# ZackAttack614/BlackBird

Measured on AMD Instinct MI355X. Metric: selfplay_games_per_sec, higher is better.
Workload: dtype f32 (float32 operands split exactly into 3 bf16 values, 6 bf16 MFMA products each, f32 accumulate)

## Files before the change

blackbird_amd/csrc/mega2.hip.h:

```cpp
#pragma once
#include "net.hip.h"
#include "net_x3.hip.h"
#include "tree.hip.h"

#define MEGA_RMAX 4
#define MEGA_HEAD_FLOATS 192

#define MEGA2_QCAP 32
#ifndef BB_TREE_IDLE_SLEEP
#define BB_TREE_IDLE_SLEEP 4
#endif
#ifndef BB_NET_IDLE_SLEEP
#define BB_NET_IDLE_SLEEP 4
#endif

__device__ __forceinline__ int lds_load(volatile int *p) { return *p; }
__device__ __forceinline__ void release_global_then_lds() {
    __threadfence_block();
    asm volatile("s_waitcnt vmcnt(0)" ::: "memory");
}


#define BB_QUEUE_SHADOWED(B, R) BB_SLOTS_TREE(B, B, R) BB_SLOTS_MAILBOX(B, B) BB_SLOTS_RESUME(B)
#define BB_QUEUE_COPY_ORDER(X)                                                                                           \
    X(root) X(root_N) X(n_nodes) X(ply) X(sims_left) X(pend_leaf) X(pend_expand) X(path_len) X(game_lid) X(sim_serial)   \
    X(leaf_serial) X(resume_cur) X(resume_depth) X(leaf_game_id) X(root_W) X(eval_value) X(eval_policy) X(evals) X(ctr)  \
    X(path) X(root_pp) X(leaf_flags)
#define BB_QUEUE_COPY_ORDER_REC(X) X(path_N) X(path_all) X(path_W)
#define BB_COUNT(...) +1
#define BB_SHADOW_PER(f) ((int)(sizeof(f) / sizeof(f[0])) / GW)
template <class G, int GW, bool REC>
struct GameShadow {
    static constexpr int S = G::S, MP = G::MAXPATH, PS = S;
#define X(T, f, per) T f[REC ? GW * (per) : 1];
    BB_QUEUE_SHADOWED(BB_SHADOW_MEMBER, X)
#undef X
    typename G::State leaf_state[GW];
    static_assert(0 BB_QUEUE_COPY_ORDER(BB_COUNT) BB_QUEUE_COPY_ORDER_REC(BB_COUNT) == 0 BB_QUEUE_SHADOWED(BB_COUNT, BB_COUNT), "a row is not copied");
    __device__ __forceinline__ void load(const TreeDev &d, int g0, int n, int nthreads) {
#define X(f) BB_SHADOW_LOAD(d, f, BB_SHADOW_PER(f))
        BB_QUEUE_COPY_ORDER(X)
        if constexpr (REC) { BB_QUEUE_COPY_ORDER_REC(X) }
#undef X
        for (int i = threadIdx.x; i < n; i += nthreads) leaf_state[i] = ((const typename G::State *)d.leaf_state)[g0 + i];
    }
    __device__ __forceinline__ void store(const TreeDev &d, int g0, int n, int nthreads) {
#define X(f) BB_SHADOW_STORE(d, f, BB_SHADOW_PER(f))
        BB_QUEUE_COPY_ORDER(X)
        if constexpr (REC) { BB_QUEUE_COPY_ORDER_REC(X) }
#undef X
        for (int i = threadIdx.x; i < n; i += nthreads) ((typename G::State *)d.leaf_state)[g0 + i] = leaf_state[i];
    }
    __device__ __forceinline__ TreeDev local(const TreeDev &d, int g0) {
        TreeDev r = d;
#define X(f) r.f = f;
        BB_QUEUE_COPY_ORDER(X)
        if constexpr (REC) { BB_QUEUE_COPY_ORDER_REC(X) }
#undef X
        r.leaf_state = leaf_state;
        r.pool_g0 = g0;
        return r;
    }
};

struct QueueCtl {
    int q[MEGA2_QCAP];
    int head, tail, tree_done, abort_flag;
};

__device__ __attribute__((noinline)) int queue_pop(QueueCtl *c, long long t_start, long long t_limit, int n_tree) {
    int li = -1;
    if ((threadIdx.x & 63) == 0) {
        int h = lds_load(&c->head), t = lds_load(&c->tail);
        if (h < t) {
            if (atomicCAS(&c->head, h, h + 1) == h) {
                volatile int *slot = &c->q[h & (MEGA2_QCAP - 1)];
                for (int spin = 0; spin < (1 << 20) && (li = *slot) < 0; spin++) __builtin_amdgcn_s_sleep(1);
                *slot = -1;
                if (li < 0) {
                    c->abort_flag = 1;
                    li = -2;
// ... 296 lines not shown
```

blackbird_amd/csrc/tree.hip.h:

```cpp
#pragma once
#include "games.hip.h"
#include "rng.hip.h"

#define NODE_EXPANDED 1
#define NODE_TERMINAL 2
#define NODE_CACHED 4
#define LEAF_RECORDED 0x40000000
#define CHILD_NONE (-1)
#define CHILD_TERM_BIT 0x40000000

template <class G>
struct alignas(128) DenseNode {
    int32_t flags;
    uint32_t legal_mask;
    int32_t all;
    int32_t serial;
    double sq;
    double pad0;
    int32_t N[G::S];
    float Q[G::S];
    int32_t child[G::S];
    alignas(128) double cP[G::S];
    float W[G::S];
    typename G::State st;
};

struct ExampleHdr {
    uint32_t game_id;
    uint16_t ply;
    uint8_t player;
    int8_t z;
    uint32_t total;
    uint32_t n_children;
};

#define BB_SLOTS_TREE(B, Q, R)                                                                     \
    B(int32_t, root, 1) B(int32_t, root_N, 1) B(int32_t, n_nodes, 1) B(int32_t, ply, 1) B(int32_t, sims_left, 1)           \
    B(int32_t, pend_leaf, 1) B(int32_t, pend_expand, 1) B(int32_t, path_len, 1)                                            \
    B(int32_t, game_lid, 1)                                             \
    B(int32_t, sim_serial, 1) B(float, root_W, 1)                                                                          \
    B(int8_t, root_pp, 1)                                   \
    B(uint32_t, path, MP)                                                                \
        \
    R(int32_t, path_N, MP) R(int32_t, path_all, MP)       \
    R(float, path_W, MP)                                                               \
    Q(int32_t, leaf_flags, 1)
#define BB_SLOTS_ANC(X)                                                                                 \
       \
    X(uint32_t, anc, ANC)                                                                                                   \
    X(int32_t, anc_len, 1) X(int32_t, top_N, 1)
#define BB_SLOTS_MAILBOX(B, Q)                                                 \
    B(uint32_t, leaf_game_id, 1) B(int32_t, leaf_serial, 1) B(float, eval_value, 1) Q(float, eval_policy, PS)              \
    B(uint64_t, evals, 1)                                                              \
    B(uint64_t, ctr, 8)
#define BB_SLOTS_OUT(X)                                                       \
    X(int32_t, out_action, 1) X(int32_t, out_root_plays, 1) X(int32_t, out_child_plays, S)                                 \
    X(float, out_root_winrate, 1) X(float, out_child_value, S)
#define BB_SLOTS_RESUME(X) X(int32_t, resume_cur, 1) X(int32_t, resume_depth, 1)
#define BB_SLOTS_POST(X) X(int, post_slot, 1)
#define BB_ROW_NONE(...)
#define BB_SLOT_ARRAYS(X) BB_SLOTS_TREE(X, X, X) BB_SLOTS_ANC(X) BB_SLOTS_MAILBOX(X, X) BB_SLOTS_OUT(X) BB_SLOTS_RESUME(X) BB_SLOTS_POST(X)
#define BB_SLOT_SHADOWED(X) BB_SLOTS_TREE(X, BB_ROW_NONE, BB_ROW_NONE) BB_SLOTS_MAILBOX(X, BB_ROW_NONE)
#define BB_SLOT_POINTER(T, f, per) T *f;
#define BB_SHADOW_MEMBER(T, f, per) T f[GW * (per)];
#define BB_SHADOW_LOAD(o, f, per) for (int i = threadIdx.x; i < n * (per); i += nthreads) f[i] = o.f[(size_t)g0 * (per) + i];
#define BB_SHADOW_STORE(o, f, per) for (int i = threadIdx.x; i < n * (per); i += nthreads) o.f[(size_t)g0 * (per) + i] = f[i];

struct TreeDev {
    int n_slots, node_cap, sims_per_move, max_plies, kind, max_depth, evaluator, priors_ones;
    int salt_per_game, max_games;
    int gpw;
    double c_puct;
    uint64_t seed, salt;
    uint32_t first_game_id;
    BB_SLOTS_TREE(BB_SLOT_POINTER, BB_SLOT_POINTER, BB_SLOT_POINTER)
    int track_anc;
    BB_SLOTS_ANC(BB_SLOT_POINTER)
    void *leaf_state;
    BB_SLOTS_MAILBOX(BB_SLOT_POINTER, BB_SLOT_POINTER)
    void *nodes;
    int n_games_target;
    double temp;
    uint8_t *examples;
    int32_t *game_hdr;
    int example_bytes;
    BB_SLOTS_OUT(BB_SLOT_POINTER)
    const double *in_u;
    BB_SLOTS_RESUME(BB_SLOT_POINTER)
    int *post_count;
    BB_SLOTS_POST(BB_SLOT_POINTER)
    int level_budget;
    int slot_offset;
    int lid_stride;
    int pool_g0;
    int *visit_pool;
    float noise_alpha;
    void *eval_cache;
    int eval_cache_log2;
// ... 30 lines not shown
#pragma unroll
    for (int k = 0; k < A; k++) a[k] = __shfl(x, k, S);
    if (A < 8) {
        double res = 0.;
#pragma unroll
        for (int k = 0; k < A; k++) res += a[k];
        return res;
    } else {
        double r[8];
#pragma unroll
        for (int j = 0; j < 8; j++) r[j] = a[j];
        int i = 8;
        for (; i < A - (A % 8); i += 8)
            for (int j = 0; j < 8; j++) r[j] += a[i + j];
        double res = ((r[0] + r[1]) + (r[2] + r[3])) + ((r[4] + r[5]) + (r[6] + r[7]));
        for (; i < A; i++) res += a[i];
        return res;
    }
}

template <int S, int STEP>
__device__ __forceinline__ void argmax_step(double &u, int &idx, int &payload) {
    double ou = dpp_step_d<STEP>(u);
    int oi = dpp_step_i<STEP>(idx), op = dpp_step_i<STEP>(payload);
    if (ou > u || (ou == u && oi < idx)) {
        u = ou;
        idx = oi;
        payload = op;
    }
}
template <int S>
__device__ __forceinline__ int grp_argmax(double u, int idx, int &payload) {
    (void)idx;
    double m = u;
    m = __builtin_fmax(m, dpp_step_d<0>(m));
    m = __builtin_fmax(m, dpp_step_d<1>(m));
    m = __builtin_fmax(m, dpp_step_d<2>(m));
    if (S == 16) m = __builtin_fmax(m, dpp_step_d<3>(m));
    const unsigned long long eq = __ballot(u == m);
    const int l64 = (int)__lane_id();
    const unsigned grp = (unsigned)(eq >> (l64 & ~(S - 1))) & ((1u << S) - 1u);
    const int win = __ffs(grp) - 1;
    payload = __shfl(payload, win, S);
    return win;
}

__device__ __forceinline__ double puct_score(double q, double cPi, double sq, int Ni, bool legal) {
    double u = q + __ddiv_rn(cPi * sq, 1.0 + (double)Ni);
    return legal ? u : -1.0;
}
#ifndef BB_PUCT_FILTER
#define BB_PUCT_FILTER 1
#endif
template <int S>
__device__ __forceinline__ int grp_argmax_puct(float qf, double cPi, double sq, int Ni, bool legal, int &payload) {
#if BB_PUCT_FILTER
    const float num = (float)(cPi * sq);
    const float uf = legal ? __builtin_fmaf(num, __builtin_amdgcn_rcpf((float)(Ni + 1)), qf) : -1.0f;
    float mf = uf;
    mf = __builtin_fmaxf(mf, __int_as_float(dpp_step_i<0>(__float_as_int(mf))));
    mf = __builtin_fmaxf(mf, __int_as_float(dpp_step_i<1>(__float_as_int(mf))));
    mf = __builtin_fmaxf(mf, __int_as_float(dpp_step_i<2>(__float_as_int(mf))));
    if (S == 16) mf = __builtin_fmaxf(mf, __int_as_float(dpp_step_i<3>(__float_as_int(mf))));
    const bool mine = uf >= mf - mf * 0x1p-18f && uf >= 0.0f;
    const unsigned long long cand = __ballot(mine);
    const int l64 = (int)__lane_id();
    const unsigned grp = (unsigned)(cand >> (l64 & ~(S - 1))) & ((1u << S) - 1u);
    if (__ballot((grp & (grp - 1u)) != 0u || grp == 0u) == 0ull) {
        const int win = __ffs(grp) - 1;
        int p = mine ? payload : 0;
        p |= dpp_step_i<0>(p);
        p |= dpp_step_i<1>(p);
        p |= dpp_step_i<2>(p);
        if (S == 16) p |= dpp_step_i<3>(p);
        payload = p;
        return win;
    }
#endif
    return grp_argmax<S>(puct_score((double)qf, cPi, sq, Ni, legal), 0, payload);
}
__device__ __forceinline__ double child_q(const TreeDev &d, float Qi, float Wi, int Ni) {
    if (d.evaluator != 2) return (double)Qi;
    return Ni > 0 ? (double)Wi / (double)Ni : 0.0;
}

template <class G>
__device__ __forceinline__ void backup_path(const TreeDev &d, int g, int lane, DenseNode<G> *pool, int plen, float v01,
                                            int prev) {
    constexpr int S = G::S;
    float vflip = 1.0f - v01;
    const uint32_t *path = d.path + (size_t)g * G::MAXPATH;
    auto edge = [&](uint32_t e) __attribute__((always_inline)) {
        int a = e & 15, pl = (e >> 4) & 3;
        DenseNode<G> *pn = pool + (e >> 6);
        int n = pn->N[a] + 1, all = pn->all + 1;
        float w = pn->W[a] + ((pl == prev) ? v01 : vflip);
        pn->N[a] = n;
        pn->W[a] = w;
        pn->Q[a] = __fdiv_rn(w, (float)n);
        pn->all = all;
        pn->sq = __dsqrt_rn(1.0 + (double)all);
    };
    for (int k = lane; k < plen; k += S) edge(path[k]);
    if (d.track_anc) {
        const uint32_t *anc = d.anc + (size_t)g * (d.max_plies + 2);
        const int na = d.anc_len[g];
        for (int k = lane; k < na; k += S) edge(anc[k]);
        if (lane == 0) d.top_N[g] += 1;
    }
    if (lane == 0) {
        d.root_N[g] += 1;
        int pp = d.root_pp[g];
        if (pp) d.root_W[g] += (pp == prev) ? v01 : vflip;
    }
}

template <class G>
__device__ __forceinline__ void phase_apply(const TreeDev &d, int g, int lane) {
    using Node = DenseNode<G>;
    constexpr int S = G::S, A = G::A;
    int leaf = d.pend_leaf[g];
    if (leaf < 0) return;
    Node *pool = (Node *)d.nodes + (size_t)(g + d.pool_g0) * d.node_cap;
    Node *node = pool + leaf;
    typename G::State st = ((const typename G::State *)d.leaf_state)[g];
    float v = d.eval_value[g];
    if (d.pend_expand[g]) {
        uint32_t mask = G::legal_mask(st);
        double x = 0.0;
        if (lane < A) x = (double)d.eval_policy[(size_t)g * S + lane] * (double)((mask >> lane) & 1u);
        double tot = grp_np_sum<A, S>(x);
        node->N[lane] = 0;
        node->Q[lane] = 0.f;
        node->W[lane] = 0.f;
        node->child[lane] = CHILD_NONE;
        node->cP[lane] = (lane < A) ? d.c_puct * __ddiv_rn(x, tot) : 0.0;
        if (lane == 0) {
            node->flags |= NODE_EXPANDED;
            node->legal_mask = mask;
            node->all = 0;
            node->sq = 1.0;
        }
    }
    int player = gs_player(st), prev = gs_prev(st);
    float v01;
    if (d.evaluator == 2) {
        v01 = v;
    } else {
        v01 = (v + 1.0f) * 0.5f;
        if (player != prev) v01 = 1.0f - v01;
    }
    if (d.evaluator != 2 && !d.pend_expand[g] && (node->flags & NODE_TERMINAL) && lane == 0) {
        node->pad0 = (double)v01;
        node->flags |= NODE_CACHED;
    }
    backup_path<G>(d, g, lane, pool, d.path_len[g], v01, prev);
    if (lane == 0) d.pend_leaf[g] = -1;
}

template <class G>
__device__ __forceinline__ void backup_path_rec(const TreeDev &d, int g, int lane, DenseNode<G> *pool, int plen, float v01, int prev) {
    constexpr int S = G::S;
    const float vflip = 1.0f - v01;
    const uint32_t *path = d.path + (size_t)g * G::MAXPATH;
    const int32_t *pN = d.path_N + (size_t)g * G::MAXPATH, *pA = d.path_all + (size_t)g * G::MAXPATH;
    const float *pW = d.path_W + (size_t)g * G::MAXPATH;
    for (int k = lane; k < plen; k += S) {
        const uint32_t e = path[k];
        const int a = e & 15, pl = (e >> 4) & 3;
        DenseNode<G> *pn = pool + (e >> 6);
        const int n = pN[k] + 1, all = pA[k] + 1;
        const float w = pW[k] + ((pl == prev) ? v01 : vflip);
        pn->N[a] = n;
        pn->W[a] = w;
        pn->Q[a] = __fdiv_rn(w, (float)n);
        pn->all = all;
        pn->sq = __dsqrt_rn(1.0 + (double)all);
    }
    if (lane == 0) {
        d.root_N[g] += 1;
        int pp = d.root_pp[g];
        if (pp) d.root_W[g] += (pp == prev) ? v01 : vflip;
    }
}

template <class G>
__device__ __forceinline__ void phase_apply_rec(const TreeDev &d, int g, int lane) {
    using Node = DenseNode<G>;
    constexpr int S = G::S, A = G::A;
    const int leaf = d.pend_leaf[g];
    if (leaf < 0) return;
    const int lf = d.leaf_flags[g] & ~LEAF_RECORDED;
    Node *pool = (Node *)d.nodes + (size_t)(g + d.pool_g0) * d.node_cap;
    Node *node = pool + leaf;
    const typename G::State st = ((const typename G::State *)d.leaf_state)[g];
    const float v = d.eval_value[g];
    const int expand = d.pend_expand[g];
    if (expand) {
        const uint32_t mask = G::legal_mask(st);
        double x = 0.0;
        if (lane < A) x = (double)d.eval_policy[(size_t)g * S + lane] * (double)((mask >> lane) & 1u);
        const double tot = grp_np_sum<A, S>(x);
        node->N[lane] = 0;
        node->Q[lane] = 0.f;
        node->W[lane] = 0.f;
        node->child[lane] = CHILD_NONE;
        node->cP[lane] = (lane < A) ? d.c_puct * __ddiv_rn(x, tot) : 0.0;
        if (lane == 0) {
            node->flags = lf | NODE_EXPANDED;
            node->legal_mask = mask;
            node->all = 0;
            node->sq = 1.0;
        }
    }
    const int player = gs_player(st), prev = gs_prev(st);
    float v01 = (v + 1.0f) * 0.5f;
    if (player != prev) v01 = 1.0f - v01;
    if (!expand && (lf & NODE_TERMINAL) && lane == 0) {
        node->pad0 = (double)v01;
        node->flags = lf | NODE_CACHED;
    }
    backup_path_rec<G>(d, g, lane, pool, d.path_len[g], v01, prev);
    if (lane == 0) d.pend_leaf[g] = -1;
}

template <class G>
__device__ __forceinline__ int create_child(const TreeDev &d, int g, DenseNode<G> *pool, DenseNode<G> *parent,
                                            const typename G::State &pst, int a, int lane, int &nn,
                                            typename G::State &st2, bool &terminal, int *flags_out = nullptr) {
    int idx = nn;
    st2 = pst;
    G::apply(st2, a);
    int w = G::winner(st2, a);
    terminal = w >= 0;
    if (idx >= d.node_cap) return CHILD_NONE;
    int word = idx | (terminal ? CHILD_TERM_BIT : 0);
    nn = idx + 1;
    const int cflags = (terminal ? (NODE_TERMINAL | ((w + 1) << 8)) : 0) | (gs_player(st2) << 4);
    if (flags_out) *flags_out = cflags;
    if (lane == 0) {
        DenseNode<G> *c = pool + idx;
        c->st = st2;
        c->flags = cflags;
        c->legal_mask = 0;
        c->all = 0;
        c->serial = idx;
        parent->child[a] = word;
        d.n_nodes[g] = idx + 1;
        d.ctr[(size_t)g * 8 + 2] += 1;
    }
    return word;
}

template <class G>
__device__ __forceinline__ uint32_t expand_ones(const TreeDev &d, DenseNode<G> *node, const typename G::State &st,
                                                int lane, double &cPi) {
    uint32_t mask = G::legal_mask(st);
    cPi = (lane < G::A && ((mask >> lane) & 1u)) ? d.c_puct * 1.0 : 0.0;
    node->N[lane] = 0;
    node->Q[lane] = 0.f;
    node->W[lane] = 0.f;
    node->child[lane] = CHILD_NONE;
    node->cP[lane] = cPi;
    if (lane == 0) {
        node->flags |= NODE_EXPANDED;
        node->legal_mask = mask;
        node->all = 0;
        node->sq = 1.0;
    }
    return mask;
}

template <class G>
__device__ void phase_select(const TreeDev &d, int g, int lane) {
    using Node = DenseNode<G>;
    constexpr int S = G::S, A = G::A;
    if (d.game_lid[g] < 0 || d.sims_left[g] <= 0) return;
    Node *pool = (Node *)d.nodes + (size_t)(g + d.pool_g0) * d.node_cap;
    uint32_t *path = d.path + (size_t)g * G::MAXPATH;
    int cur = d.root[g];
    int nn = d.n_nodes[g];
    int depth = 0, expand = 0, overflow = 0, term_leaf = 0;
    const bool inline_expand = d.priors_ones != 0;
    const bool fixed = d.kind == 1, rollout = d.evaluator == 2;
    typename G::State st;
    int flags = 0;
    bool have = false;
#ifdef BB_STAMPS
    long long acc_load = 0, acc_iter = 0;
#endif
    for (int it = 0;; it++) {
#ifdef BB_STAMPS
        long long ts0 = clock64();
        acc_iter++;
#endif
        Node *node = pool + cur;
        typename G::State st_l = node->st;
        int flags_l = node->flags;
        uint32_t mask = node->legal_mask;
        double sq = node->sq;
        int Ni = node->N[lane];
        float Qi = node->Q[lane];
        float Wi = rollout ? node->W[lane] : 0.f;
        double cPi = node->cP[lane];
        int ci = node->child[lane];
        asm volatile("" ::"v"(flags_l), "v"(mask), "v"(sq), "v"(Ni), "v"(Qi), "v"(cPi), "v"(ci));
#ifdef BB_STAMPS
        acc_load += clock64() - ts0;
#endif
        if (!have) {
            st = st_l;
            flags = flags_l;
        }
        have = false;
        if (fixed && it >= d.max_depth) break;
        if (!(flags & NODE_EXPANDED)) {
            if (flags & NODE_TERMINAL) { term_leaf = 1; break; }
            if (!inline_expand) { expand = 1; break; }
            mask = expand_ones<G>(d, node, st, lane, cPi);
            if (!fixed) break;
            Ni = 0;
            Qi = 0.f;
            Wi = 0.f;
            sq = 1.0;
            ci = CHILD_NONE;
        }
        if (mask == 0) break;
        double u = puct_score(child_q(d, Qi, Wi, Ni), cPi, sq, Ni, lane < A && ((mask >> lane) & 1u));
        int child = ci;
        int a = grp_argmax<S>(u, lane, child);
        if (depth >= G::MAXPATH) { overflow = 1; break; }
        if (child == CHILD_NONE) {
            typename G::State st2;
            bool terminal;
            child = create_child<G>(d, g, pool, node, st, a, lane, nn, st2, terminal);
            if (child == CHILD_NONE) { overflow = 1; break; }
            if (lane == 0) path[depth] = ((uint32_t)cur << 6) | ((uint32_t)((flags >> 4) & 3) << 4) | (uint32_t)a;
            st = st2;
            flags = (terminal ? NODE_TERMINAL : 0) | (gs_player(st2) << 4);
            have = true;
        } else {
            if (lane == 0) path[depth] = ((uint32_t)cur << 6) | ((uint32_t)((flags >> 4) & 3) << 4) | (uint32_t)a;
        }
        depth++;
        cur = child & ~CHILD_TERM_BIT;
    }
#ifdef BB_STAMPS
    if (d.stamps && lane == 0) {
        atomicAdd(&d.stamps[5], (unsigned long long)acc_load);
        atomicAdd(&d.stamps[6], (unsigned long long)acc_iter);
        atomicAdd(&d.stamps[7], 1ull);
    }
#endif
    if (lane == 0) {
        ((typename G::State *)d.leaf_state)[g] = st;
        d.leaf_game_id[g] = d.first_game_id + (uint32_t)d.game_lid[g];
        d.leaf_serial[g] = cur;
        d.pend_leaf[g] = cur;
// ... 8 lines not shown
        c[1] += (uint64_t)depth;
        c[3] += (uint64_t)term_leaf;
        c[6] += (uint64_t)overflow;
    }
}

template <class G>
__global__ void __launch_bounds__(256) k_tree_step(TreeDev d) {
    constexpr int S = G::S;
    int t = blockIdx.x * blockDim.x + threadIdx.x;
    int wv = t >> 6, l64 = t & 63;
    if (l64 >= d.gpw * S) return;
    int g = wv * d.gpw + l64 / S, lane = l64 % S;
    if (g >= d.n_slots) return;
#ifdef BB_STAMPS
    long long t0 = clock64();
#endif
    phase_apply<G>(d, g, lane);
#ifdef BB_STAMPS
    long long t1 = clock64();
#endif
    __threadfence_block();
#ifdef BB_STAMPS
    long long t2 = clock64();
#endif
    phase_select<G>(d, g, lane);
#ifdef BB_STAMPS
    long long t3 = clock64();
    if ((threadIdx.x & 63) == 0 && d.stamps) {
        atomicAdd(&d.stamps[0], (unsigned long long)(t1 - t0));
        atomicAdd(&d.stamps[1], (unsigned long long)(t2 - t1));
        atomicAdd(&d.stamps[2], (unsigned long long)(t3 - t2));
        atomicAdd(&d.stamps[4], 1ull);
    }
#endif
}

template <class G>
__global__ void __launch_bounds__(256) k_tree_apply(TreeDev d) {
    constexpr int S = G::S;
    int t = blockIdx.x * blockDim.x + threadIdx.x;
    int g = t / S, lane = t % S;
    if (g >= d.n_slots) return;
    phase_apply<G>(d, g, lane);
}

template <class G>
__device__ __forceinline__ int choose_move(const TreeDev &d, int g, int lane, double temp, double u, int &total, int &Ni_out,
                           float &Wi_out) {
    using Node = DenseNode<G>;
    constexpr int S = G::S, A = G::A;
    Node *pool = (Node *)d.nodes + (size_t)(g + d.pool_g0) * d.node_cap;
    Node *node = pool + d.root[g];
    if (!(node->flags & NODE_EXPANDED)) {
        total = 0;
        Ni_out = 0;
        Wi_out = 0.f;
        return -3;
    }
    uint32_t mask = node->legal_mask;
    bool legal = lane < A && ((mask >> lane) & 1u);
    int Ni = legal ? node->N[lane] : 0;
    float Wi = legal ? node->W[lane] : 0.f;
    Ni_out = Ni;
    Wi_out = Wi;
    int all = grp_sum_i<S>(Ni);
    total = all;
    if (temp == 0.0) {
        double uu = puct_score(child_q(d, node->Q[lane], Wi, Ni), node->cP[lane], node->sq, Ni, legal);
        int dummy = 0;
        return grp_argmax<S>(uu, lane, dummy);
    }
    double it = 1.0 / temp;
    double w = (it == 1.0) ? (double)Ni : pow((double)Ni, it);
    double ws[A];
#pragma unroll
    for (int k = 0; k < A; k++) ws[k] = __shfl(w, k, S);
    double allp = 0.0;
#pragma unroll
    for (int k = 0; k < A; k++) allp += ws[k];
    if (!(allp > 0.0)) return -4;
    double last = 0.0;
#pragma unroll
    for (int k = 0; k < A; k++) last += __ddiv_rn(ws[k], allp);
    double run = 0.0;
    int act = A - 1;
    bool found = false;
#pragma unroll
    for (int k = 0; k < A; k++) {
        run += __ddiv_rn(ws[k], allp);
        if (!found && __ddiv_rn(run, last) > u) {
            act = k;
            found = true;
        }
    }
    return act;
}

template <class G>
__global__ void __launch_bounds__(256) k_sample(TreeDev d, double temp) {
    constexpr int S = G::S;
    int t = blockIdx.x * blockDim.x + threadIdx.x;
    int g = t / S, lane = t % S;
    if (g >= d.n_slots) return;
    if (d.game_lid[g] < 0) {
        if (lane == 0 && d.out_action) d.out_action[g] = -3;
        return;
    }
    double u = d.in_u ? d.in_u[g] : bb_u53(d.seed, d.first_game_id + (uint32_t)d.game_lid[g], (uint32_t)d.ply[g]);
    int total, Ni;
    float Wi;
    int act = choose_move<G>(d, g, lane, temp, u, total, Ni, Wi);
    if (d.out_child_plays) d.out_child_plays[(size_t)g * S + lane] = Ni;
    if (d.out_child_value) d.out_child_value[(size_t)g * S + lane] = Wi;
    if (lane == 0) {
        if (d.out_action) d.out_action[g] = act;
        if (d.out_root_plays) d.out_root_plays[g] = d.root_N[g];
        if (d.out_root_winrate) {
            int n = d.root_N[g];
            float w = d.root_W[g];
            d.out_root_winrate[g] = n > 0 ? ((d.evaluator == 2) ? (float)((double)w / (double)n) : __fdiv_rn(w, (float)n)) : 0.f;
        }
    }
}

template <class G>
__device__ __forceinline__ void advance_root(const TreeDev &d, int g, int lane, int a, typename G::State &new_st) {
    using Node = DenseNode<G>;
    Node *pool = (Node *)d.nodes + (size_t)(g + d.pool_g0) * d.node_cap;
    Node *node = pool + d.root[g];
    typename G::State st = node->st;
    if (!(node->flags & NODE_EXPANDED)) {
        new_st = st;
        G::apply(new_st, a);
        if (lane == 0) {
            Node *r = pool;
            r->st = new_st;
            r->flags = gs_player(new_st) << 4;
            r->serial = 0;
            d.n_nodes[g] = 1;
            d.root[g] = 0;
            d.root_N[g] = 0;
            d.root_W[g] = 0.f;
            d.root_pp[g] = 0;
            if (d.track_anc) {
                d.anc_len[g] = 0;
                d.top_N[g] = 0;
            }
        }
        return;
    }
    int child = node->child[a];
    int cn = node->N[a];
    float cw = node->W[a];
    if (child == CHILD_NONE) {
        bool terminal;
        int nn = d.n_nodes[g];
        child = create_child<G>(d, g, pool, node, st, a, lane, nn, new_st, terminal);
        if (child == CHILD_NONE) {
            child = 0;
            cn = 0;
            cw = 0.f;
            if (lane == 0) {
                pool->st = new_st;
                pool->flags = gs_player(new_st) << 4;
                d.n_nodes[g] = 1;
                d.ctr[(size_t)g * 8 + 6] += 1;
            }
        }
    } else {
        new_st = pool[child & ~CHILD_TERM_BIT].st;
    }
    if (lane == 0) {
        if (d.track_anc) {
            if (child == 0 && cn == 0 && d.n_nodes[g] == 1) {
                d.anc_len[g] = 0;
                d.top_N[g] = 0;
            } else if (d.anc_len[g] < d.max_plies + 2) {
                d.anc[(size_t)g * (d.max_plies + 2) + d.anc_len[g]] = ((uint32_t)d.root[g] << 6) | ((uint32_t)gs_player(st) << 4) | (uint32_t)a;
                d.anc_len[g] += 1;
            }
        }
        d.root[g] = child & ~CHILD_TERM_BIT;
        d.root_N[g] = cn;
        d.root_W[g] = cw;
        d.root_pp[g] = (int8_t)gs_player(st);
    }
}

template <class G>
__global__ void __launch_bounds__(256) k_reset_roots(TreeDev d) {
    int g = blockIdx.x * blockDim.x + threadIdx.x;
    if (g >= d.n_slots || !d.track_anc || d.game_lid[g] < 0 || d.anc_len[g] <= 0) return;
    d.root[g] = (int)(d.anc[(size_t)g * (d.max_plies + 2)] >> 6);
    d.root_N[g] = d.top_N[g];
    d.root_W[g] = 0.f;
    d.root_pp[g] = 0;
    d.anc_len[g] = 0;
}

template <class G>
__global__ void __launch_bounds__(64) k_node_view(TreeDev d, int g, int node, int32_t *child_out, int32_t *plays_out, float *value_out,
                                                   typename G::State *state_out, int32_t *info_out) {
    using Node = DenseNode<G>;
    const int lane = threadIdx.x;
    if (lane >= G::S) return;
    Node *pool = (Node *)d.nodes + (size_t)(g + d.pool_g0) * d.node_cap;
    if (node < 0) node = d.root[g];
    const Node *n = pool + node;
    const bool exp = (n->flags & NODE_EXPANDED) != 0;
    child_out[lane] = exp ? n->child[lane] : CHILD_NONE;
    plays_out[lane] = exp ? n->N[lane] : 0;
    value_out[lane] = exp ? n->W[lane] : 0.f;
    if (lane == 0) {
        *state_out = n->st;
        info_out[0] = n->flags;
        info_out[1] = (int32_t)(exp ? n->legal_mask : 0u);
        info_out[2] = node;
    }
}

template <class G>
__global__ void __launch_bounds__(256) k_move_roots(TreeDev d, const int32_t *actions) {
    constexpr int S = G::S;
    int t = blockIdx.x * blockDim.x + threadIdx.x;
    int g = t / S, lane = t % S;
    if (g >= d.n_slots) return;
    int a = actions[g];
    if (a < 0 || a >= G::A || d.game_lid[g] < 0) return;
    typename G::State ns;
    advance_root<G>(d, g, lane, a, ns);
    if (lane == 0) d.ply[g] += 1;
}

template <class G>
__device__ __forceinline__ void reset_slot(const TreeDev &d, int g, int lid, const typename G::State &st) {
    using Node = DenseNode<G>;
    Node *pool = (Node *)d.nodes + (size_t)(g + d.pool_g0) * d.node_cap;
    pool->st = st;
    pool->flags = gs_player(st) << 4;
    pool->legal_mask = 0;
    pool->all = 0;
    pool->serial = 0;
    d.n_nodes[g] = 1;
    d.root[g] = 0;
    d.root_N[g] = 0;
    d.root_W[g] = 0.f;
    d.root_pp[g] = 0;
    d.ply[g] = 0;
    d.pend_leaf[g] = -1;
    d.pend_expand[g] = 0;
    d.path_len[g] = 0;
    d.sim_serial[g] = 0;
    d.game_lid[g] = lid;
    if (d.leaf_flags) d.leaf_flags[g] = 0;
    if (d.track_anc) {
        d.anc_len[g] = 0;
        d.top_N[g] = 0;
    }
}

template <class G>
__global__ void __launch_bounds__(256) k_set_roots(TreeDev d, int n, const int32_t *slots,
                                                   const typename G::State *states, const uint32_t *game_ids) {
    int i = blockIdx.x * blockDim.x + threadIdx.x;
    if (i >= n) return;
    int g = slots ? slots[i] : i;
    if (g < 0 || g >= d.n_slots) return;
    reset_slot<G>(d, g, game_ids ? (int)game_ids[i] : g, states[i]);
    d.sims_left[g] = 0;
}

template <class G>
__global__ void __launch_bounds__(256) k_add_sims(TreeDev d, int sims, const uint8_t *mask = nullptr) {
    int g = blockIdx.x * blockDim.x + threadIdx.x;
    if (g >= d.n_slots) return;
    if (d.game_lid[g] >= 0 && (!mask || mask[g])) d.sims_left[g] = sims;
}

template <class G>
__global__ void __launch_bounds__(256) k_get_roots(TreeDev d, typename G::State *out) {
    int g = blockIdx.x * blockDim.x + threadIdx.x;
    if (g >= d.n_slots) return;
    out[g] = ((DenseNode<G> *)d.nodes + (size_t)(g + d.pool_g0) * d.node_cap + d.root[g])->st;
}

template <class G>
__global__ void __launch_bounds__(256) k_selfplay_begin(TreeDev d) {
    int g = blockIdx.x * blockDim.x + threadIdx.x;
    if (g >= d.n_slots) return;
    if (g + d.slot_offset < d.n_games_target) {
        reset_slot<G>(d, g, g + d.slot_offset, G::initial());
        d.sims_left[g] = d.sims_per_move;
    } else {
        reset_slot<G>(d, g, -1, G::initial());
        d.sims_left[g] = 0;
// ... 88 lines not shown
    }
}

template <class G>
__global__ void __launch_bounds__(256) k_selfplay_move(TreeDev d) {
    constexpr int S = G::S;
    int t = blockIdx.x * blockDim.x + threadIdx.x;
    int g = t / S, lane = t % S;
    if (g >= d.n_slots) return;
    phase_apply<G>(d, g, lane);
    __threadfence_block();
    selfplay_move_body<G>(d, g, lane);
}

struct NoPostHook {
    __device__ __forceinline__ void operator()(int, int) const {}
};
template <class G, bool REC = false, class OnPost = NoPostHook>
__device__ bool async_game(const TreeDev &d, int g, int lane
#ifdef BB_STAMPS_LIGHT
                           , int &g_light_loop, int &g_light_levels, int &g_light_load, int &g_light_puct
#endif
                           , OnPost on_post = OnPost()) {
    using Node = DenseNode<G>;
    constexpr int S = G::S, A = G::A;
    if (d.game_lid[g] < 0) return false;
    Node *pool = (Node *)d.nodes + (size_t)(g + d.pool_g0) * d.node_cap;
#ifdef BB_STAMPS_LIGHT
    int lt_in = (int)clock64(), lt_loop = 0, ln_levels = 0, lt_create = 0, lt_puct = 0;
#endif
    if (d.pend_leaf[g] >= 0) {
        if (REC && (d.leaf_flags[g] & LEAF_RECORDED)) phase_apply_rec<G>(d, g, lane);
        else phase_apply<G>(d, g, lane);
        if (lane == 0) d.sims_left[g] -= 1;
        __threadfence_block();
    }
    int budget = d.level_budget;
    uint32_t *path = d.path + (size_t)g * G::MAXPATH;
    int sims_done = 0, depth_sum = 0, term_hits = 0;
    bool posted = false;
    for (;;) {
        if (d.sims_left[g] <= 0) {
            selfplay_move_body<G>(d, g, lane);
            __threadfence_block();
            if (d.game_lid[g] < 0) break;
        }
        int cur = d.resume_cur[g], depth = 0;
        if (cur >= 0) depth = d.resume_depth[g];
        else cur = d.root[g];
        int nn = d.n_nodes[g];
        typename G::State st;
        int flags = 0;
        enum { F_PARKED = 2, F_LEAF = 4, F_TERM = 8, F_EXPAND = 16, F_OVERFLOW = 32 };
        int fl = 0;
#ifdef BB_STAMPS_LIGHT
        int lt_e = (int)clock64();
#endif
        for (;;) {
            if (budget <= 0) { fl |= F_PARKED; break; }
            budget--;
#ifdef BB_STAMPS_LIGHT
            ln_levels++;
            int lt_a = (int)clock64();
#endif
            Node *node = pool + cur;
            typename G::State st_l = node->st;
            int flags_l = node->flags;
            uint32_t mask = node->legal_mask;
            double sq = node->sq;
            int Ni = node->N[lane];
            float Qi = node->Q[lane];
            double cPi = node->cP[lane];
            int ci = node->child[lane];
            double cached = node->pad0;
            float Wi = 0.f;
            int all_l = 0;
            if (REC) {
                Wi = node->W[lane];
                all_l = node->all;
            }
            asm volatile("" ::"v"(flags_l), "v"(mask), "v"(sq), "v"(Ni), "v"(Qi), "v"(cPi), "v"(ci));
#ifdef BB_STAMPS_LIGHT
            int lt_b = (int)clock64();
            lt_create += lt_b - lt_a;
#endif
            st = st_l;
            flags = flags_l;
            if (!(flags & NODE_EXPANDED)) {
                fl |= F_LEAF;
                if (flags & NODE_TERMINAL) {
                    fl |= F_TERM;
                    if (flags & NODE_CACHED) {
                        float v01 = (float)cached;
                        __threadfence_block();
                        if (REC) backup_path_rec<G>(d, g, lane, pool, depth, v01, gs_prev(st));
                        else backup_path<G>(d, g, lane, pool, depth, v01, gs_prev(st));
                        if (lane == 0) d.sims_left[g] -= 1;
                        __threadfence_block();
                        sims_done++;
                        depth_sum += depth;
                        term_hits++;
                        fl &= ~F_LEAF;
                    }
                } else {
                    fl |= F_EXPAND;
                }
                break;
            }
            static_assert(G::MAXPATH >= G::H * G::W + 2, "a descent places at most H*W stones");
            int child = ci;
            int a = grp_argmax_puct<S>(Qi, cPi, sq, Ni, lane < A && ((mask >> lane) & 1u), child);
#ifdef BB_STAMPS_LIGHT
            asm volatile("" ::"v"(a), "v"(child));
            lt_puct += (int)clock64() - lt_b;
#endif
            if (lane == 0) path[depth] = ((uint32_t)cur << 6) | ((uint32_t)((flags >> 4) & 3) << 4) | (uint32_t)a;
            if (REC) {
                if (lane == 0) d.path_all[(size_t)g * G::MAXPATH + depth] = all_l;
                if (lane == a) {
                    d.path_N[(size_t)g * G::MAXPATH + depth] = Ni;
                    d.path_W[(size_t)g * G::MAXPATH + depth] = Wi;
                }
            }
            if (child == CHILD_NONE) {
                typename G::State st2;
                bool terminal;
                child = create_child<G>(d, g, pool, node, st, a, lane, nn, st2, terminal, &flags);
                if (child == CHILD_NONE) { fl |= F_OVERFLOW | F_LEAF; break; }
                st = st2;
                depth++;
                cur = child & ~CHILD_TERM_BIT;
                fl |= F_LEAF | (terminal ? F_TERM : F_EXPAND);
                break;
            }
            depth++;
            cur = child & ~CHILD_TERM_BIT;
        }
#ifdef BB_STAMPS_LIGHT
        lt_loop += (int)clock64() - lt_e;
#endif
        if (lane == 0) {
            d.resume_cur[g] = (fl & F_PARKED) ? cur : -1;
            d.resume_depth[g] = (fl & F_PARKED) ? depth : 0;
        }
        if (fl & F_PARKED) break;
        if (!(fl & F_LEAF)) {
            if (lane == 0) d.sim_serial[g] += 1;
            continue;
        }
        if (lane == 0) {
            ((typename G::State *)d.leaf_state)[g] = st;
            d.leaf_game_id[g] = d.first_game_id + (uint32_t)d.game_lid[g];
            d.leaf_serial[g] = cur;
            d.pend_leaf[g] = cur;
            if (d.leaf_flags) d.leaf_flags[g] = REC ? (flags | LEAF_RECORDED) : 0;
            d.pend_expand[g] = (fl & F_EXPAND) ? 1 : 0;
            d.path_len[g] = depth;
            d.sim_serial[g] += 1;
            d.evals[g] += 1;
            d.ctr[(size_t)g * 8 + 6] += (uint64_t)((fl & F_OVERFLOW) ? 1 : 0);
        }
        on_post(g, lane);
        sims_done++;
        depth_sum += depth;
        term_hits += (fl & F_TERM) ? 1 : 0;
        posted = true;
        break;
    }
#ifdef BB_STAMPS_LIGHT
    g_light_loop = lt_loop;
    g_light_load = lt_create;
    g_light_puct = lt_puct;
    g_light_levels = ln_levels;
    (void)lt_in;
#endif
    if (lane == 0 && sims_done) {
        uint64_t *c = d.ctr + (size_t)g * 8;
        c[0] += (uint64_t)sims_done;
        c[1] += (uint64_t)depth_sum;
        c[3] += (uint64_t)term_hits;
    }
    return posted;
}

template <class G>
__global__ void __launch_bounds__(256) k_tree_async(TreeDev d, int round) {
    constexpr int S = G::S;
    int t = blockIdx.x * blockDim.x + threadIdx.x;
    int wv = t >> 6, l64 = t & 63;
// ... 30 lines not shown
```

Measured before the change: 9355.

## Pack node edges and header into one cache line; defer state loads in descent

New measurement: 9621 (median of 6 runs). +2.8%, better.

```diff
diff --git a/blackbird_amd/csrc/mega2.hip.h b/blackbird_amd/csrc/mega2.hip.h
--- a/blackbird_amd/csrc/mega2.hip.h
+++ b/blackbird_amd/csrc/mega2.hip.h
@@ -26,7 +26,7 @@
     X(root) X(root_N) X(n_nodes) X(ply) X(sims_left) X(pend_leaf) X(pend_expand) X(path_len) X(game_lid) X(sim_serial)   \
     X(leaf_serial) X(resume_cur) X(resume_depth) X(leaf_game_id) X(root_W) X(eval_value) X(eval_policy) X(evals) X(ctr)  \
     X(path) X(root_pp) X(leaf_flags)
-#define BB_QUEUE_COPY_ORDER_REC(X) X(path_N) X(path_all) X(path_W)
+#define BB_QUEUE_COPY_ORDER_REC(X) X(path_rec)
 #define BB_COUNT(...) +1
 #define BB_SHADOW_PER(f) ((int)(sizeof(f) / sizeof(f[0])) / GW)
 template <class G, int GW, bool REC>
diff --git a/blackbird_amd/csrc/tree.hip.h b/blackbird_amd/csrc/tree.hip.h
--- a/blackbird_amd/csrc/tree.hip.h
+++ b/blackbird_amd/csrc/tree.hip.h
@@ -9,20 +9,49 @@
 #define CHILD_NONE (-1)
 #define CHILD_TERM_BIT 0x40000000
 
+struct alignas(16) NodeEdge {
+    int32_t N;
+    float Q;
+    int32_t child;
+    float cPf;
+};
+struct alignas(16) NodeHead {
+    int32_t flags;
+    union {
+        uint32_t legal_mask;
+        int32_t term_prev;
+    };
+    int32_t all;
+    union {
+        float sqf;
+        float term_v01;
+    };
+};
+union NodeSlot {
+    NodeEdge e;
+    NodeHead h;
+};
 template <class G>
 struct alignas(128) DenseNode {
-    int32_t flags;
-    uint32_t legal_mask;
-    int32_t all;
-    int32_t serial;
-    double sq;
-    double pad0;
-    int32_t N[G::S];
-    float Q[G::S];
-    int32_t child[G::S];
+    static_assert(G::A < G::S, "the last child slot of a row carries its header");
+    NodeSlot s[G::S];
     alignas(128) double cP[G::S];
     float W[G::S];
     typename G::State st;
+    double sq;
+    __host__ __device__ NodeEdge &e(int i) { return s[i].e; }
+    __host__ __device__ const NodeEdge &e(int i) const { return s[i].e; }
+    __host__ __device__ NodeHead &h() { return s[G::S - 1].h; }
+    __host__ __device__ const NodeHead &h() const { return s[G::S - 1].h; }
+};
+static_assert(sizeof(DenseNode<Connect4>) == 256 && sizeof(DenseNode<TicTacToe>) == 512, "node rows keep their size: pool sizing (bb_fit_slots)");
+static_assert(offsetof(DenseNode<Connect4>, cP) == 128, "Connect4: a level reads one 128-byte line");
+
+struct alignas(16) PathRec {
+    uint32_t e;
+    int32_t all;
+    int32_t N;
+    float W;
 };
 
 struct ExampleHdr {
@@ -41,9 +70,8 @@
     B(int32_t, sim_serial, 1) B(float, root_W, 1)                                                                          \
     B(int8_t, root_pp, 1)                                   \
     B(uint32_t, path, MP)                                                                \
-        \
-    R(int32_t, path_N, MP) R(int32_t, path_all, MP)       \
-    R(float, path_W, MP)                                                               \
+           \
+    R(PathRec, path_rec, MP)                                                                                               \
     Q(int32_t, leaf_flags, 1)
 #define BB_SLOTS_ANC(X)                                                                                 \
        \
@@ -180,10 +208,10 @@
 #ifndef BB_PUCT_FILTER
 #define BB_PUCT_FILTER 1
 #endif
-template <int S>
-__device__ __forceinline__ int grp_argmax_puct(float qf, double cPi, double sq, int Ni, bool legal, int &payload) {
+template <int S, class Node>
+__device__ __forceinline__ int grp_argmax_puct(float qf, float cPf, float sqf, int Ni, bool legal, int &payload, const Node *node, int lane) {
 #if BB_PUCT_FILTER
-    const float num = (float)(cPi * sq);
+    const float num = cPf * sqf;
     const float uf = legal ? __builtin_fmaf(num, __builtin_amdgcn_rcpf((float)(Ni + 1)), qf) : -1.0f;
     float mf = uf;
     mf = __builtin_fmaxf(mf, __int_as_float(dpp_step_i<0>(__float_as_int(mf))));
@@ -205,7 +233,7 @@
         return win;
     }
 #endif
-    return grp_argmax<S>(puct_score((double)qf, cPi, sq, Ni, legal), 0, payload);
+    return grp_argmax<S>(puct_score((double)qf, node->cP[lane], node->sq, Ni, legal), 0, payload);
 }
 __device__ __forceinline__ double child_q(const TreeDev &d, float Qi, float Wi, int Ni) {
     if (d.evaluator != 2) return (double)Qi;
@@ -214,22 +242,25 @@
 
 template <class G>
 __device__ __forceinline__ void backup_path(const TreeDev &d, int g, int lane, DenseNode<G> *pool, int plen, float v01,
-                                            int prev) {
+                                            int prev, bool recd = false) {
     constexpr int S = G::S;
     float vflip = 1.0f - v01;
-    const uint32_t *path = d.path + (size_t)g * G::MAXPATH;
+    const uint32_t *path = recd ? &d.path_rec[(size_t)(g + d.pool_g0) * G::MAXPATH].e : d.path + (size_t)g * G::MAXPATH;
+    const int pstride = recd ? (int)(sizeof(PathRec) / sizeof(uint32_t)) : 1;
     auto edge = [&](uint32_t e) __attribute__((always_inline)) {
         int a = e & 15, pl = (e >> 4) & 3;
         DenseNode<G> *pn = pool + (e >> 6);
-        int n = pn->N[a] + 1, all = pn->all + 1;
+        int n = pn->e(a).N + 1, all = pn->h().all + 1;
         float w = pn->W[a] + ((pl == prev) ? v01 : vflip);
-        pn->N[a] = n;
+        const double sq = __dsqrt_rn(1.0 + (double)all);
+        pn->e(a).N = n;
+        pn->e(a).Q = __fdiv_rn(w, (float)n);
         pn->W[a] = w;
-        pn->Q[a] = __fdiv_rn(w, (float)n);
-        pn->all = all;
-        pn->sq = __dsqrt_rn(1.0 + (double)all);
+        pn->h().all = all;
+        pn->h().sqf = (float)sq;
+        pn->sq = sq;
     };
-    for (int k = lane; k < plen; k += S) edge(path[k]);
+    for (int k = lane; k < plen; k += S) edge(path[k * pstride]);
     if (d.track_anc) {
         const uint32_t *anc = d.anc + (size_t)g * (d.max_plies + 2);
         const int na = d.anc_len[g];
@@ -258,17 +289,14 @@
         double x = 0.0;
         if (lane < A) x = (double)d.eval_policy[(size_t)g * S + lane] * (double)((mask >> lane) & 1u);
         double tot = grp_np_sum<A, S>(x);
-        node->N[lane] = 0;
-        node->Q[lane] = 0.f;
+        const double cPi = (lane < A) ? d.c_puct * __ddiv_rn(x, tot) : 0.0;
+        NodeSlot sl;
+        if (lane < S - 1) sl.e = NodeEdge{0, 0.f, CHILD_NONE, (float)cPi};
+        else sl.h = NodeHead{node->h().flags | NODE_EXPANDED, {mask}, 0, {1.0f}};
+        node->s[lane] = sl;
         node->W[lane] = 0.f;
-        node->child[lane] = CHILD_NONE;
-        node->cP[lane] = (lane < A) ? d.c_puct * __ddiv_rn(x, tot) : 0.0;
-        if (lane == 0) {
-            node->flags |= NODE_EXPANDED;
-            node->legal_mask = mask;
-            node->all = 0;
-            node->sq = 1.0;
-        }
+        node->cP[lane] = cPi;
+        if (lane == 0) node->sq = 1.0;
     }
     int player = gs_player(st), prev = gs_prev(st);
     float v01;
@@ -278,11 +306,11 @@
         v01 = (v + 1.0f) * 0.5f;
         if (player != prev) v01 = 1.0f - v01;
     }
-    if (d.evaluator != 2 && !d.pend_expand[g] && (node->flags & NODE_TERMINAL) && lane == 0) {
-        node->pad0 = (double)v01;
-        node->flags |= NODE_CACHED;
-    }
-    backup_path<G>(d, g, lane, pool, d.path_len[g], v01, prev);
+    if (d.evaluator != 2 && !d.pend_expand[g] && (node->h().flags & NODE_TERMINAL) && lane == 0) {
+        node->h().term_v01 = v01;
+        node->h().flags |= NODE_CACHED;
+    }
+    backup_path<G>(d, g, lane, pool, d.path_len[g], v01, prev, d.leaf_flags && (d.leaf_flags[g] & LEAF_RECORDED));
     if (lane == 0) d.pend_leaf[g] = -1;
 }
 
@@ -290,20 +318,20 @@
 __device__ __forceinline__ void backup_path_rec(const TreeDev &d, int g, int lane, DenseNode<G> *pool, int plen, float v01, int prev) {
     constexpr int S = G::S;
     const float vflip = 1.0f - v01;
-    const uint32_t *path = d.path + (size_t)g * G::MAXPATH;
-    const int32_t *pN = d.path_N + (size_t)g * G::MAXPATH, *pA = d.path_all + (size_t)g * G::MAXPATH;
-    const float *pW = d.path_W + (size_t)g * G::MAXPATH;
+    const PathRec *rec = d.path_rec + (size_t)g * G::MAXPATH;
     for (int k = lane; k < plen; k += S) {
-        const uint32_t e = path[k];
-        const int a = e & 15, pl = (e >> 4) & 3;
-        DenseNode<G> *pn = pool + (e >> 6);
-        const int n = pN[k] + 1, all = pA[k] + 1;
-        const float w = pW[k] + ((pl == prev) ? v01 : vflip);
-        pn->N[a] = n;
+        const PathRec r = rec[k];
+        const int a = r.e & 15, pl = (r.e >> 4) & 3;
+        DenseNode<G> *pn = pool + (r.e >> 6);
+        const int n = r.N + 1, all = r.all + 1;
+        const float w = r.W + ((pl == prev) ? v01 : vflip);
+        const double sq = __dsqrt_rn(1.0 + (double)all);
+        pn->e(a).N = n;
+        pn->e(a).Q = __fdiv_rn(w, (float)n);
         pn->W[a] = w;
-        pn->Q[a] = __fdiv_rn(w, (float)n);
-        pn->all = all;
-        pn->sq = __dsqrt_rn(1.0 + (double)all);
+        pn->h().all = all;
+        pn->h().sqf = (float)sq;
+        pn->sq = sq;
     }
     if (lane == 0) {
         d.root_N[g] += 1;
@@ -329,24 +357,21 @@
         double x = 0.0;
         if (lane < A) x = (double)d.eval_policy[(size_t)g * S + lane] * (double)((mask >> lane) & 1u);
         const double tot = grp_np_sum<A, S>(x);
-        node->N[lane] = 0;
-        node->Q[lane] = 0.f;
+        const double cPi = (lane < A) ? d.c_puct * __ddiv_rn(x, tot) : 0.0;
+        NodeSlot sl;
+        if (lane < S - 1) sl.e = NodeEdge{0, 0.f, CHILD_NONE, (float)cPi};
+        else sl.h = NodeHead{lf | NODE_EXPANDED, {mask}, 0, {1.0f}};
+        node->s[lane] = sl;
         node->W[lane] = 0.f;
-        node->child[lane] = CHILD_NONE;
-        node->cP[lane] = (lane < A) ? d.c_puct * __ddiv_rn(x, tot) : 0.0;
-        if (lane == 0) {
-            node->flags = lf | NODE_EXPANDED;
-            node->legal_mask = mask;
-            node->all = 0;
-            node->sq = 1.0;
-        }
+        node->cP[lane] = cPi;
+        if (lane == 0) node->sq = 1.0;
     }
     const int player = gs_player(st), prev = gs_prev(st);
     float v01 = (v + 1.0f) * 0.5f;
     if (player != prev) v01 = 1.0f - v01;
     if (!expand && (lf & NODE_TERMINAL) && lane == 0) {
-        node->pad0 = (double)v01;
-        node->flags = lf | NODE_CACHED;
+        node->h().term_v01 = v01;
+        node->h().flags = lf | NODE_CACHED;
     }
     backup_path_rec<G>(d, g, lane, pool, d.path_len[g], v01, prev);
     if (lane == 0) d.pend_leaf[g] = -1;
@@ -369,11 +394,8 @@
     if (lane == 0) {
         DenseNode<G> *c = pool + idx;
         c->st = st2;
-        c->flags = cflags;
-        c->legal_mask = 0;
-        c->all = 0;
-        c->serial = idx;
-        parent->child[a] = word;
+        c->h() = NodeHead{cflags, {terminal ? (uint32_t)gs_prev(st2) : 0u}, 0, {0.f}};
+        parent->e(a).child = word;
         d.n_nodes[g] = idx + 1;
         d.ctr[(size_t)g * 8 + 2] += 1;
     }
@@ -385,17 +407,13 @@
                                                 int lane, double &cPi) {
     uint32_t mask = G::legal_mask(st);
     cPi = (lane < G::A && ((mask >> lane) & 1u)) ? d.c_puct * 1.0 : 0.0;
-    node->N[lane] = 0;
-    node->Q[lane] = 0.f;
+    NodeSlot sl;
+    if (lane < G::S - 1) sl.e = NodeEdge{0, 0.f, CHILD_NONE, (float)cPi};
+    else sl.h = NodeHead{node->h().flags | NODE_EXPANDED, {mask}, 0, {1.0f}};
+    node->s[lane] = sl;
     node->W[lane] = 0.f;
-    node->child[lane] = CHILD_NONE;
     node->cP[lane] = cPi;
-    if (lane == 0) {
-        node->flags |= NODE_EXPANDED;
-        node->legal_mask = mask;
-        node->all = 0;
-        node->sq = 1.0;
-    }
+    if (lane == 0) node->sq = 1.0;
     return mask;
 }
 
@@ -424,14 +442,16 @@
 #endif
         Node *node = pool + cur;
         typename G::State st_l = node->st;
-        int flags_l = node->flags;
-        uint32_t mask = node->legal_mask;
+        const NodeSlot mine_l = node->s[lane];
+        const NodeHead head_l = node->h();
+        int flags_l = head_l.flags;
+        uint32_t mask = head_l.legal_mask;
         double sq = node->sq;
-        int Ni = node->N[lane];
-        float Qi = node->Q[lane];
+        int Ni = mine_l.e.N;
+        float Qi = mine_l.e.Q;
         float Wi = rollout ? node->W[lane] : 0.f;
         double cPi = node->cP[lane];
-        int ci = node->child[lane];
+        int ci = mine_l.e.child;
         asm volatile("" ::"v"(flags_l), "v"(mask), "v"(sq), "v"(Ni), "v"(Qi), "v"(cPi), "v"(ci));
 #ifdef BB_STAMPS
         acc_load += clock64() - ts0;
@@ -546,22 +566,22 @@
     constexpr int S = G::S, A = G::A;
     Node *pool = (Node *)d.nodes + (size_t)(g + d.pool_g0) * d.node_cap;
     Node *node = pool + d.root[g];
-    if (!(node->flags & NODE_EXPANDED)) {
+    if (!(node->h().flags & NODE_EXPANDED)) {
         total = 0;
         Ni_out = 0;
         Wi_out = 0.f;
         return -3;
     }
-    uint32_t mask = node->legal_mask;
+    uint32_t mask = node->h().legal_mask;
     bool legal = lane < A && ((mask >> lane) & 1u);
-    int Ni = legal ? node->N[lane] : 0;
+    int Ni = legal ? node->e(lane).N : 0;
     float Wi = legal ? node->W[lane] : 0.f;
     Ni_out = Ni;
     Wi_out = Wi;
     int all = grp_sum_i<S>(Ni);
     total = all;
     if (temp == 0.0) {
-        double uu = puct_score(child_q(d, node->Q[lane], Wi, Ni), node->cP[lane], node->sq, Ni, legal);
+        double uu = puct_score(child_q(d, legal ? node->e(lane).Q : 0.f, Wi, Ni), node->cP[lane], node->sq, Ni, legal);
         int dummy = 0;
         return grp_argmax<S>(uu, lane, dummy);
     }
@@ -624,14 +644,13 @@
     Node *pool = (Node *)d.nodes + (size_t)(g + d.pool_g0) * d.node_cap;
     Node *node = pool + d.root[g];
     typename G::State st = node->st;
-    if (!(node->flags & NODE_EXPANDED)) {
+    if (!(node->h().flags & NODE_EXPANDED)) {
         new_st = st;
         G::apply(new_st, a);
         if (lane == 0) {
             Node *r = pool;
             r->st = new_st;
-            r->flags = gs_player(new_st) << 4;
-            r->serial = 0;
+            r->h() = NodeHead{gs_player(new_st) << 4, {0u}, 0, {0.f}};
             d.n_nodes[g] = 1;
             d.root[g] = 0;
             d.root_N[g] = 0;
@@ -644,8 +663,8 @@
         }
         return;
     }
-    int child = node->child[a];
-    int cn = node->N[a];
+    int child = node->e(a).child;
+    int cn = node->e(a).N;
     float cw = node->W[a];
     if (child == CHILD_NONE) {
         bool terminal;
@@ -657,7 +676,7 @@
             cw = 0.f;
             if (lane == 0) {
                 pool->st = new_st;
-                pool->flags = gs_player(new_st) << 4;
+                pool->h() = NodeHead{gs_player(new_st) << 4, {0u}, 0, {0.f}};
                 d.n_nodes[g] = 1;
                 d.ctr[(size_t)g * 8 + 6] += 1;
             }
@@ -702,14 +721,14 @@
     Node *pool = (Node *)d.nodes + (size_t)(g + d.pool_g0) * d.node_cap;
     if (node < 0) node = d.root[g];
     const Node *n = pool + node;
-    const bool exp = (n->flags & NODE_EXPANDED) != 0;
-    child_out[lane] = exp ? n->child[lane] : CHILD_NONE;
-    plays_out[lane] = exp ? n->N[lane] : 0;
-    value_out[lane] = exp ? n->W[lane] : 0.f;
+    const bool exp = (n->h().flags & NODE_EXPANDED) != 0, slot = exp && lane < G::S - 1;
+    child_out[lane] = slot ? n->e(lane).child : CHILD_NONE;
+    plays_out[lane] = slot ? n->e(lane).N : 0;
+    value_out[lane] = slot ? n->W[lane] : 0.f;
     if (lane == 0) {
         *state_out = n->st;
-        info_out[0] = n->flags;
-        info_out[1] = (int32_t)(exp ? n->legal_mask : 0u);
+        info_out[0] = n->h().flags;
+        info_out[1] = (int32_t)(exp ? n->h().legal_mask : 0u);
         info_out[2] = node;
     }
 }
@@ -732,10 +751,7 @@
     using Node = DenseNode<G>;
     Node *pool = (Node *)d.nodes + (size_t)(g + d.pool_g0) * d.node_cap;
     pool->st = st;
-    pool->flags = gs_player(st) << 4;
-    pool->legal_mask = 0;
-    pool->all = 0;
-    pool->serial = 0;
+    pool->h() = NodeHead{gs_player(st) << 4, {0u}, 0, {0.f}};
     d.n_nodes[g] = 1;
     d.root[g] = 0;
     d.root_N[g] = 0;
@@ -930,89 +946,87 @@
         typename G::State st;
         int flags = 0;
         enum { F_PARKED = 2, F_LEAF = 4, F_TERM = 8, F_EXPAND = 16, F_OVERFLOW = 32 };
-        int fl = 0;
+        int fl = F_PARKED;
+        Node *node = pool + cur;
+        NodeHead head = {};
 #ifdef BB_STAMPS_LIGHT
         int lt_e = (int)clock64();
 #endif
-        for (;;) {
-            if (budget <= 0) { fl |= F_PARKED; break; }
-            budget--;
+        PathRec pend = {};
+        int pend_a = -1;
+        for (; budget > 0; budget--) {
 #ifdef BB_STAMPS_LIGHT
             ln_levels++;
             int lt_a = (int)clock64();
 #endif
-            Node *node = pool + cur;
-            typename G::State st_l = node->st;
-            int flags_l = node->flags;
-            uint32_t mask = node->legal_mask;
-            double sq = node->sq;
-            int Ni = node->N[lane];
-            float Qi = node->Q[lane];
-            double cPi = node->cP[lane];
-            int ci = node->child[lane];
-            double cached = node->pad0;
-            float Wi = 0.f;
-            int all_l = 0;
-            if (REC) {
-                Wi = node->W[lane];
-                all_l = node->all;
-            }
-            asm volatile("" ::"v"(flags_l), "v"(mask), "v"(sq), "v"(Ni), "v"(Qi), "v"(cPi), "v"(ci));
+            node = pool + cur;
+            const NodeSlot mine_l = node->s[lane];
+            head = node->h();
+            int Ni = mine_l.e.N;
+            float Qi = mine_l.e.Q, cPf = mine_l.e.cPf;
+            int ci = mine_l.e.child;
+            asm volatile("" ::"v"(head.flags), "v"(head.legal_mask), "v"(head.sqf), "v"(Ni), "v"(Qi), "v"(cPf), "v"(ci));
 #ifdef BB_STAMPS_LIGHT
             int lt_b = (int)clock64();
             lt_create += lt_b - lt_a;
 #endif
-            st = st_l;
-            flags = flags_l;
-            if (!(flags & NODE_EXPANDED)) {
-                fl |= F_LEAF;
-                if (flags & NODE_TERMINAL) {
-                    fl |= F_TERM;
-                    if (flags & NODE_CACHED) {
-                        float v01 = (float)cached;
-                        __threadfence_block();
-                        if (REC) backup_path_rec<G>(d, g, lane, pool, depth, v01, gs_prev(st));
-                        else backup_path<G>(d, g, lane, pool, depth, v01, gs_prev(st));
-                        if (lane == 0) d.sims_left[g] -= 1;
-                        __threadfence_block();
-                        sims_done++;
-                        depth_sum += depth;
-                        term_hits++;
-                        fl &= ~F_LEAF;
-                    }
-                } else {
-                    fl |= F_EXPAND;
-                }
+            if (REC && lane == pend_a) d.path_rec[(size_t)g * G::MAXPATH + depth - 1] = pend;
+            if (!(head.flags & NODE_EXPANDED)) {
+                fl = 0;
+                pend_a = -1;
                 break;
             }
             static_assert(G::MAXPATH >= G::H * G::W + 2, "a descent places at most H*W stones");
             int child = ci;
-            int a = grp_argmax_puct<S>(Qi, cPi, sq, Ni, lane < A && ((mask >> lane) & 1u), child);
+            const int a = grp_argmax_puct<S>(Qi, cPf, head.sqf, Ni, lane < A && ((head.legal_mask >> lane) & 1u), child, node, lane);
 #ifdef BB_STAMPS_LIGHT
             asm volatile("" ::"v"(a), "v"(child));
             lt_puct += (int)clock64() - lt_b;
 #endif
-            if (lane == 0) path[depth] = ((uint32_t)cur << 6) | ((uint32_t)((flags >> 4) & 3) << 4) | (uint32_t)a;
+            const uint32_t pw = ((uint32_t)cur << 6) | ((uint32_t)((head.flags >> 4) & 3) << 4) | (uint32_t)a;
             if (REC) {
-                if (lane == 0) d.path_all[(size_t)g * G::MAXPATH + depth] = all_l;
-                if (lane == a) {
-                    d.path_N[(size_t)g * G::MAXPATH + depth] = Ni;
-                    d.path_W[(size_t)g * G::MAXPATH + depth] = Wi;
-                }
+                pend = PathRec{pw, head.all, Ni, node->W[a]};
+                pend_a = a;
+            } else {
+                if (lane == 0) path[depth] = pw;
             }
             if (child == CHILD_NONE) {
-                typename G::State st2;
-                bool terminal;
-                child = create_child<G>(d, g, pool, node, st, a, lane, nn, st2, terminal, &flags);
-                if (child == CHILD_NONE) { fl |= F_OVERFLOW | F_LEAF; break; }
-                st = st2;
-                depth++;
-                cur = child & ~CHILD_TERM_BIT;
-                fl |= F_LEAF | (terminal ? F_TERM : F_EXPAND);
+                fl = F_EXPAND | a << 8;
                 break;
             }
             depth++;
             cur = child & ~CHILD_TERM_BIT;
+        }
+        flags = head.flags;
+        if (fl & F_EXPAND) st = node->st;
+        if (REC && lane == pend_a) d.path_rec[(size_t)g * G::MAXPATH + ((fl & F_EXPAND) ? depth : depth - 1)] = pend;
+        if (fl & F_EXPAND) {
+            typename G::State st2;
+            bool terminal;
+            const int child = create_child<G>(d, g, pool, node, st, fl >> 8, lane, nn, st2, terminal, &flags);
+            if (child == CHILD_NONE) {
+                fl = F_OVERFLOW | F_LEAF;
+            } else {
+                st = st2;
+                depth++;
+                cur = child & ~CHILD_TERM_BIT;
+                fl = F_LEAF | (terminal ? F_TERM : F_EXPAND);
+            }
+        } else if (!(fl & F_PARKED)) {
+            if ((flags & (NODE_TERMINAL | NODE_CACHED)) == (NODE_TERMINAL | NODE_CACHED)) {
+                __threadfence_block();
+                if (REC) backup_path_rec<G>(d, g, lane, pool, depth, head.term_v01, head.term_prev);
+                else backup_path<G>(d, g, lane, pool, depth, head.term_v01, head.term_prev);
+                if (lane == 0) d.sims_left[g] -= 1;
+                __threadfence_block();
+                sims_done++;
+                depth_sum += depth;
+                term_hits++;
+                fl = F_TERM;
+            } else {
+                st = node->st;
+                fl = F_LEAF | ((flags & NODE_TERMINAL) ? F_TERM : F_EXPAND);
+            }
         }
 #ifdef BB_STAMPS_LIGHT
         lt_loop += (int)clock64() - lt_e;
```
